# jackBonadies/Guided-Attention

Hardware: AMD Instinct MI355X
Metric: guided images/sec (50-step SD-1.5 512^2) (higher is better)
Workload: dtype f16

## Files before the change

guided-attention_amd/_lib.py:

```python
import ctypes
import os
from pathlib import Path

import torch

_HERE = Path(__file__).resolve().parent
LIB_PATH = Path(os.environ.get("GA_HIP_LIB", _HERE / "libga_hip.so"))

GA_VERSION = 182
GA_F16, GA_BF16, GA_F32 = 0, 1, 2
GA_LINEAR_STREAM = 8
GA_TOK_COOR, GA_TOK_BOX = 0, 1
GA_TERMS = 8
GA_MAX_IMAGES = 64
GA_IMAGE_MAX_TOKENS = 32
DTYPE_CODE = {torch.float16: GA_F16, torch.bfloat16: GA_BF16, torch.float32: GA_F32}


class GaError(RuntimeError):
    pass


class ga_token_t(ctypes.Structure):
    _fields_ = [("token", ctypes.c_int32), ("kind", ctypes.c_int32), ("geom", ctypes.c_double * 4),
                ("weight", ctypes.c_float), ("_pad", ctypes.c_float)]


class ga_loss_params_t(ctypes.Structure):
    _fields_ = [("inside_scale", ctypes.c_float), ("outside_scale", ctypes.c_float), ("center_weight", ctypes.c_float),
                ("sigma", ctypes.c_float), ("shrink", ctypes.c_double), ("ksize", ctypes.c_int32),
                ("smooth", ctypes.c_int32), ("strict", ctypes.c_int32), ("_pad", ctypes.c_int32)]

# ... 56 lines not shown
    "ga_bias_residual_add": [_vp, _vp, _vp, _vp, _i64, _i, _i, _vp],
    "ga_cat_channels": [_vp, _vp, _vp, _i64, _i, _i, _i, _vp],
    "ga_cat_channels_gn_blocks": [_i, _i, _i, _i],
    "ga_linear_gn_blocks": [_i, _i, _i, _i, _i],
    "ga_group_norm_one_launch": [_i, _i, _i, _i],
    "ga_cat_group_norm_fwd": [_vp, _vp, _vp, _vp, _vp, _vp, _vp, _i, _i, _i, _i, _i, _f, _i, _i, _vp],
    "ga_cat_channels_gn": [_vp, _vp, _vp, _vp, _i, _i, _i, _i, _i, _i, _vp],
    "ga_conv3x3_packed_elems": [_i, _i],
    "ga_conv3x3_thin_packed_elems": [_i, _i],
    "ga_conv3x3_thin_supported": [_i, _i, _i, _i],
    "ga_conv3x3_thin_pack": [_vp, _vp, _i, _i, _i64, _i64, _i64, _i64, _i, _i, _vp],
    "ga_conv3x3_thin_in": [_vp, _vp, _vp, _vp, _i, _i, _i, _i, _i, _vp],
    "ga_conv3x3_thin_out": [_vp, _vp, _vp, _vp, _i, _i, _i, _i, _i, _vp],
    "ga_conv3x3_pack_weights": [_vp, _vp, _i, _i, _i64, _i64, _i64, _i64, _i, _i, _vp],
    "ga_conv3x3_plan": [_i, _i, _i, _i, _i, _i, ctypes.POINTER(_i), ctypes.POINTER(_i), ctypes.POINTER(_i),
                        ctypes.POINTER(ctypes.c_longlong)],
    "ga_splitk_workspace_floats": [_i64, _i, _i, _i, _i],
    "ga_conv3x3_nhwc": [_vp, _vp, _vp, _vp, _vp, _vp, _vp, _i, _i, _i, _i, _i, _i, _i, _i, _i, _i, _vp],
    "ga_conv3x3_gn_blocks": [_i, _i, _i, _i, _i, _i],
    "ga_conv3x3_nhwc_gn": [_vp, _vp, _vp, _vp, _vp, _vp, _vp, _i, _i, _i, _i, _i, _i, _i, _i, _i, _vp, _vp, _vp, _i],
    "ga_group_norm_apply": [_vp, _vp, _vp, _vp, _vp, _vp, _vp, _i, _i, _i, _i, _i, _f, _i, _i, _vp],
    "ga_group_norm_two_launch": [_i, _i, _i, _i],
    "ga_conv3x3_up2x_nhwc": [_vp, _vp, _vp, _vp, _vp, _vp, _vp, _i, _i, _i, _i, _i, _i, _i, _i, _i, _vp],
    "ga_gemm_nt": [_vp, _vp, _vp, _vp, _vp, _vp, _vp, _i64, _i, _i, _i, _i, _i, _i, _vp],
    "ga_linear_workspace": [_i64, _i, _i, _i, _i, _i, ctypes.POINTER(ctypes.c_longlong), ctypes.POINTER(_i)],
    "ga_linear_fused": [_vp, _i64, _vp, _vp, _i64, ctypes.POINTER(ga_linear_epilogue_t), _vp, _vp, _i64, _i, _i, _i, _i, _i,
                        _i, _i, _vp],
    "ga_add_layer_norm_fwd": [_vp, _vp, _vp, _vp, _vp, _vp, _vp, _i64, _i, _f, _i, _vp],
    "ga_add_layer_norm_bwd": [_vp, _vp, _vp, _vp, _vp, _vp, _i64, _i, _i, _vp],
}

_lib = None


def load():
    global _lib
    if _lib is None:
        if not LIB_PATH.exists():
            raise GaError(f"{LIB_PATH} not found: build it with `make` (or __graft_entry__.build()); "
                          "the guided-attention path has no CPU fallback")
        lib = ctypes.CDLL(str(LIB_PATH))
        lib.ga_version.argtypes, lib.ga_version.restype = [], ctypes.c_int
        built = lib.ga_version()
        if built != GA_VERSION:
            raise GaError(f"{LIB_PATH} is ABI version {built}, this binding is written for {GA_VERSION}: rebuild with `make`")
        for name, argtypes in PROTOTYPES.items():
# ... 29 lines not shown
```

guided-attention_amd/csrc/conv3x3.hip:

```cpp
#include <cstdlib>

#include "attn_common.h"

using namespace ga;

namespace {

typedef float f32x16 __attribute__((ext_vector_type(16)));
typedef unsigned int u32x4_t __attribute__((ext_vector_type(4)));

#ifndef GA_CONV_PRIO
#define GA_CONV_PRIO 0
#endif
#ifndef GA_CONV_KC
#define GA_CONV_KC 64
#endif
#ifndef GA_CONV_ABL
#define GA_CONV_ABL 0
#endif
constexpr int kKC = GA_CONV_KC;
constexpr int kLD = kKC + 8;
constexpr int kThreads = 256;

template <typename T>
// ... 7 lines not shown
template <>
struct Mma32<bf16_t> {
  __device__ static __forceinline__ f32x16 run(uint4 a, uint4 b, f32x16 c) {
    return __builtin_amdgcn_mfma_f32_32x32x16_bf16(__builtin_bit_cast(bf16x8, a), __builtin_bit_cast(bf16x8, b), c, 0, 0, 0);
  }
};

struct ConvArgs {
  int B, H, W, Cin, Ho, Wo, Cout, stride;
  int M;
  int steps;
  int steps_per;
  int tm, tn;
  int splits;
  int n_fastest;
  int pad;
  int lane_rot;
  unsigned x_bytes, w_bytes;
  int w_tap, w_blk, w_row, w_chunk;
  int pg_nseg, pg_srows;
  int pg_dpr, pg_dpc;
  FastDiv d_tm, d_tn, d_w, d_hw, d_pw, d_segpw, d_segpx, d_wo, d_howo;
  int up;
  float* gn_partials;
  const void* gn_cbias;
  int gn_cg, gn_G, gn_tpi;
};

__device__ __forceinline__ void conv_args_resident(const ConvArgs& a) {
#if defined(__HIP_DEVICE_COMPILE__)
#define GA_TOUCH(x) asm volatile("" ::"s"(x))
  GA_TOUCH(a.B); GA_TOUCH(a.H); GA_TOUCH(a.W); GA_TOUCH(a.Cin); GA_TOUCH(a.Ho); GA_TOUCH(a.Wo); GA_TOUCH(a.Cout); GA_TOUCH(a.stride);
  GA_TOUCH(a.M); GA_TOUCH(a.steps); GA_TOUCH(a.steps_per); GA_TOUCH(a.tm); GA_TOUCH(a.tn); GA_TOUCH(a.splits); GA_TOUCH(a.n_fastest);
  GA_TOUCH(a.pad); GA_TOUCH(a.lane_rot); GA_TOUCH(a.x_bytes); GA_TOUCH(a.w_bytes);
  GA_TOUCH(a.w_tap); GA_TOUCH(a.w_blk); GA_TOUCH(a.w_row); GA_TOUCH(a.w_chunk);
  GA_TOUCH(a.pg_nseg); GA_TOUCH(a.pg_srows); GA_TOUCH(a.pg_dpr); GA_TOUCH(a.pg_dpc);
  GA_TOUCH(a.d_tm.d); GA_TOUCH(a.d_tm.m); GA_TOUCH(a.d_tn.d); GA_TOUCH(a.d_tn.m); GA_TOUCH(a.d_w.d); GA_TOUCH(a.d_w.m);
  GA_TOUCH(a.d_hw.d); GA_TOUCH(a.d_hw.m); GA_TOUCH(a.d_pw.d); GA_TOUCH(a.d_pw.m); GA_TOUCH(a.d_segpw.d); GA_TOUCH(a.d_segpw.m);
  GA_TOUCH(a.d_segpx.d); GA_TOUCH(a.d_segpx.m); GA_TOUCH(a.d_wo.d); GA_TOUCH(a.d_wo.m); GA_TOUCH(a.d_howo.d); GA_TOUCH(a.d_howo.m);
  GA_TOUCH(a.up);
#undef GA_TOUCH
#endif
}

__device__ __forceinline__ unsigned w_row_bytes(const ConvArgs& a, int n, int piece) {
  return (unsigned)(((n >> 6) * a.w_blk + (n & 63) * a.w_row + 8 * piece) * 2);
}
__device__ __forceinline__ unsigned w_step_bytes(const ConvArgs& a, int tap, int chunk) {
  return (unsigned)((tap * a.w_tap + chunk * a.w_chunk) * 2);
}

__device__ __forceinline__ int lane_pixel(int fr, int rot) { return fr < 16 || rot == 0 ? fr : 16 + ((fr - 16 - rot) & 15); }

template <int BM, int BN>
__device__ __forceinline__ void tile_of_workgroup(const ConvArgs& a, int& m0, int& n0, int& split) {
  const int total = a.tm * a.tn * a.splits, q = total >> 3, r = total & 7;
  const int xcd = blockIdx.x & 7, slot = blockIdx.x >> 3;
  const int logical = (xcd < r ? xcd * (q + 1) : r * (q + 1) + (xcd - r) * q) + slot;
  const bool nf = a.n_fastest != 0;
  const FastDiv d1 = nf ? a.d_tn : a.d_tm, d2 = nf ? a.d_tm : a.d_tn;
  const int t1 = nf ? a.tn : a.tm, t2 = nf ? a.tm : a.tn;
  const int rest = fdiv(logical, d1), i1 = logical - rest * t1;
  split = fdiv(rest, d2);
// ... 94 lines not shown
            for (int qd = 0; qd < 4; ++qd)
#pragma unroll
              for (int r = 0; r < 4; ++r)
                acc[j][i][4 * qd + r] += in ? __uint_as_float(v[sb][(j * IM + i) * 4 + qd][r]) : 0.f;
      }
    }
  }
  {
    constexpr int LDC = BN + 8;
    T* Cs = lds;
    float gsum[8] = {0.f, 0.f, 0.f, 0.f, 0.f, 0.f, 0.f, 0.f}, gsq[8] = {0.f, 0.f, 0.f, 0.f, 0.f, 0.f, 0.f, 0.f};
#pragma unroll
    for (int i = 0; i < IM; ++i)
#pragma unroll
      for (int j = 0; j < JN; ++j)
#pragma unroll
        for (int qd = 0; qd < 4; ++qd) {
          typename Traits<T>::frag f;
#pragma unroll
          for (int r = 0; r < 4; ++r) f[r] = Traits<T>::from_f32(acc[j][i][4 * qd + r]);
          store_frag<T>(Cs + (wm * WM + i * 32 + fr) * LDC + wn * WN + j * 32 + 8 * qd + 4 * fh, f);
        }
    __syncthreads();
#pragma unroll
    for (int k = 0; k < NV; ++k) {
      const int r = r0 + k * (kThreads / VPR);
      const int m = m0 + r, n = n0 + cv;
      uint4 val = *reinterpret_cast<const uint4*>(Cs + r * LDC + cv);
      if (bias != nullptr || residual != nullptr) {
        T* e = reinterpret_cast<T*>(&val);
        const T* be = reinterpret_cast<const T*>(&bvec);
        const T* re = reinterpret_cast<const T*>(&rvec[k]);
#pragma unroll
        for (int q = 0; q < 8; ++q)
          e[q] = Traits<T>::from_f32(Traits<T>::to_f32(e[q]) + Traits<T>::to_f32(be[q]) + Traits<T>::to_f32(re[q]));
      }
      if (m < a.M && n < a.Cout) *reinterpret_cast<uint4*>(Y + (size_t)m * a.Cout + n) = val;
      if (gn && m < a.M && n < a.Cout) {
        const T* e = reinterpret_cast<const T*>(&val);
        const T* ge = reinterpret_cast<const T*>(&gvec);
#pragma unroll
        for (int q = 0; q < 8; ++q) {
          const float x = Traits<T>::to_f32(e[q]) + Traits<T>::to_f32(ge[q]);
          gsum[q] += x;
          gsq[q] += x * x;
        }
// ... 61 lines not shown
  __shared__ __attribute__((aligned(16))) T lds[kLds];

  const int tid = threadIdx.x, lane = tid & 63, wave = tid >> 6;
  const int wm = wave >> 1, wn = wave & 1;
  int m0, n0, split;
  conv_args_resident(a);
  tile_of_workgroup<BM, BN>(a, m0, n0, split);
  const int it0 = split * a.steps_per, it1 = min(a.steps, it0 + a.steps_per);
  const int cchunks = a.Cin / kKC;

  constexpr unsigned kOob = 0x80000000u;
  const int srow = tid / QP, sq = tid % QP;
  int a_iy[PA], a_ix[PA];
  int a_off[PA];
#pragma unroll
  for (int p = 0; p < PA; ++p) {
    const int m = m0 + srow + RPP * p;
    const bool ok = m < a.M;
    const int mm = ok ? m : 0;
    const int b = sdiv(mm, a.d_howo), rem = mm - b * (a.Ho * a.Wo);
    const int oy = sdiv(rem, a.d_wo), ox = rem - oy * a.Wo;
    a_iy[p] = ok ? oy * a.stride - a.pad : -4;
    a_ix[p] = ox * a.stride - a.pad;
    a_off[p] = (((b * a.H + a_iy[p]) * a.W + a_ix[p]) * a.Cin + 8 * sq) * (int)sizeof(T);
  }
  unsigned b_off[PB];
#pragma unroll
  for (int p = 0; p < PB; ++p) {
    const int n = n0 + srow + RPP * p;
    b_off[p] = n < a.Cout ? w_row_bytes(a, n, sq) : kOob;
  }
  typedef unsigned int u32x4 __attribute__((ext_vector_type(4)));
  const __amdgpu_buffer_rsrc_t xrsrc = __builtin_amdgcn_make_buffer_rsrc(const_cast<T*>(X), 0, a.x_bytes, 0x00020000);
  const __amdgpu_buffer_rsrc_t wrsrc = __builtin_amdgcn_make_buffer_rsrc(const_cast<T*>(Wp), 0, a.w_bytes, 0x00020000);
  uint4 ra0[PA], rb0[PB], ra1[PA], rb1[PB];
  int ld_it = it0, ld_tap = it0 / cchunks, ld_c = it0 - ld_tap * cchunks;
  int ld_ky = ld_tap / 3, ld_kx = ld_tap - 3 * ld_ky;
  bool in_loop = false;
  auto load_step = [&](uint4 (&ra)[PA], uint4 (&rb)[PB]) {
    if ((GA_CONV_ABL & 1) && in_loop) return;
    const int a_step = ((ld_ky * a.W + ld_kx) * a.Cin + ld_c * kKC) * (int)sizeof(T);
    const unsigned b_step = w_step_bytes(a, ld_tap, ld_c);
#pragma unroll
    for (int p = 0; p < PA; ++p) {
      const bool in = (unsigned)(a_iy[p] + ld_ky) < (unsigned)a.H && (unsigned)(a_ix[p] + ld_kx) < (unsigned)a.W;
      const u32x4 x = __builtin_amdgcn_raw_buffer_load_b128(xrsrc, in ? (unsigned)(a_off[p] + a_step) : kOob, 0, 0);
      ra[p] = uint4{x[0], x[1], x[2], x[3]};
    }
#pragma unroll
    for (int p = 0; p < PB; ++p) {
      const u32x4 x = __builtin_amdgcn_raw_buffer_load_b128(wrsrc, b_off[p] + b_step, 0, 0);
      rb[p] = uint4{x[0], x[1], x[2], x[3]};
    }
    if (ld_it + 1 < it1) {
      ++ld_it;
      if (++ld_c == cchunks) {
        ld_c = 0;
        ++ld_tap;
        if (++ld_kx == 3) {
          ld_kx = 0;
          ++ld_ky;
        }
      }
    }
// ... 130 lines not shown
  if (run) {
    const int in_image = m0 - sdiv(m0, a.d_hw) * hw;
    col0 = in_image - sdiv(in_image, a.d_w) * a.W;
  }
  const int PW = a.W + 2, seg_px = (int)a.d_segpx.d, seg_rows = g.srows + 2, seg_pw = seg_rows * PW;
  const int npatch = g.nseg * seg_pw;

  constexpr unsigned kOob = 0x80000000u;
  const int srow = tid / QP, sq = tid % QP;
  typedef unsigned int u32x4 __attribute__((ext_vector_type(4)));
  const __amdgpu_buffer_rsrc_t xrsrc = __builtin_amdgcn_make_buffer_rsrc(const_cast<T*>(X), 0, a.x_bytes, 0x00020000);
  const __amdgpu_buffer_rsrc_t wrsrc = __builtin_amdgcn_make_buffer_rsrc(const_cast<T*>(Wp), 0, a.w_bytes, 0x00020000);

  unsigned pa_off[kPatchPieces];
#pragma unroll
  for (int p = 0; p < kPatchPieces; ++p) {
    const int q = srow + RPP * p;
    const int seg = sdiv(q, a.d_segpw), rem = q - seg * seg_pw;
    const int pr = sdiv(rem, a.d_pw), pc = rem - pr * PW;
    const int mseg = m0 + seg * seg_px;
    const int b = sdiv(mseg, a.d_hw), y0 = sdiv(mseg - b * hw, a.d_w);
    const int iy = y0 + pr - 1, ix = pc - 1;
    const bool ok = q < npatch && mseg < a.M && (unsigned)iy < (unsigned)a.H && (unsigned)ix < (unsigned)a.W;
    pa_off[p] = ok ? (unsigned)((((b * a.H + iy) * a.W + ix) * a.Cin + 8 * sq) * (int)sizeof(T)) : kOob;
  }
  uint4 rp[kPatchPieces];
  auto load_patch = [&](int chunk) {
    const unsigned step = (unsigned)(chunk * kKC * (int)sizeof(T));
#pragma unroll
    for (int p = 0; p < kPatchPieces; ++p) {
      const u32x4 x = __builtin_amdgcn_raw_buffer_load_b128(xrsrc, pa_off[p] + step, 0, 0);
      rp[p] = uint4{x[0], x[1], x[2], x[3]};
    }
  };
  auto store_patch = [&]() {
#pragma unroll
    for (int p = 0; p < kPatchPieces; ++p)
      *reinterpret_cast<uint4*>(patch + (srow + RPP * p) * kLD + 8 * sq) = rp[p];
  };

  unsigned b_off[PB];
#pragma unroll
  for (int p = 0; p < PB; ++p) {
    const int n = n0 + srow + RPP * p;
    b_off[p] = n < a.Cout ? w_row_bytes(a, n, sq) : kOob;
  }
  constexpr int NS = BN <= 64 ? 9 : 3, PD = BN <= 64 ? 6 : 3;
// ... 186 lines not shown

  PatchGeom g{a.pg_nseg, a.pg_srows};
  const int hw = a.H * a.W;
  const bool run = a.d_segpx.d == (unsigned)BM && BM != g.srows * a.W;
  int col0 = 0;
  if (run) {
    const int in_image = m0 - fdiv(m0, a.d_hw) * hw;
    col0 = in_image - fdiv(in_image, a.d_w) * a.W;
  }
  const int PW = a.W + 2, seg_px = (int)a.d_segpx.d, seg_rows = g.srows + 2, seg_pw = seg_rows * PW;

  constexpr unsigned kOob = 0x80000000u;
  const int srow = tid / QP, sq = tid % QP;
  const __amdgpu_buffer_rsrc_t xrsrc = __builtin_amdgcn_make_buffer_rsrc(const_cast<T*>(X), 0, a.x_bytes, 0x00020000);
  const __amdgpu_buffer_rsrc_t wrsrc = __builtin_amdgcn_make_buffer_rsrc(const_cast<T*>(Wp), 0, a.w_bytes, 0x00020000);
  const unsigned lds0 = (unsigned)(uintptr_t)((__attribute__((address_space(3))) void*)lds);

  unsigned pa_off[kPatchPieces];
  auto patch_offsets = [&]() {
    int seg = fdiv(srow, a.d_segpw);
    const int rem0 = srow - seg * seg_pw;
    int pr = fdiv(rem0, a.d_pw), pc = rem0 - pr * PW;
    const int b0 = fdiv(m0, a.d_hw), y00 = fdiv(m0 - b0 * hw, a.d_w);
    const unsigned row_bytes = (unsigned)(a.Cin * (int)sizeof(T));
    const int SH = a.up ? a.H >> 1 : a.H, SW = a.up ? a.W >> 1 : a.W;
#pragma unroll
    for (int p = 0; p < kPatchPieces; ++p) {
      const int mseg = m0 + seg * seg_px;
      const int b = b0 + seg;
      const int iy = y00 + pr - 1, ix = pc - 1;
      const bool ok = seg < g.nseg && mseg < a.M && (unsigned)iy < (unsigned)a.H && (unsigned)ix < (unsigned)a.W;
      const int sy = a.up ? iy >> 1 : iy, sx = a.up ? ix >> 1 : ix;
      const unsigned pix = __umul24(__umul24((unsigned)b, (unsigned)SH) + (unsigned)sy, (unsigned)SW) + (unsigned)sx;
      pa_off[p] = ok ? __umul24(pix, row_bytes) + (unsigned)(8 * sq * (int)sizeof(T)) : kOob;
      pc += a.pg_dpc;
      pr += a.pg_dpr;
      if (pc >= PW) { pc -= PW; ++pr; }
      if (pr >= seg_rows) { pr -= seg_rows; ++seg; }
      if (pr >= seg_rows) { pr -= seg_rows; ++seg; }
    }
  };
  u32x4_t rp[kPatchPieces];
  auto load_patch = [&](int chunk) {
    const unsigned step = (unsigned)(chunk * kKC * (int)sizeof(T));
#pragma unroll
    for (int p = 0; p < kPatchPieces; ++p) rp[p] = __builtin_amdgcn_raw_buffer_load_b128(xrsrc, pa_off[p] + step, 0, 0);
  };
  const unsigned patch_st = lds0 + (unsigned)((srow * kLD + 8 * sq) * (int)sizeof(T));
  auto store_patch = [&]() {
#pragma unroll
    for (int p = 0; p < kPatchPieces; ++p) conv_lds_write128(patch_st + (unsigned)(RPP * p * kLD * (int)sizeof(T)), rp[p]);
  };

  const int wave_u = __builtin_amdgcn_readfirstlane(wave);
// ... 213 lines not shown
  PatchGeom pg{1, 1};
  const bool geom_ok = a.pad == 1 && a.stride == 1 && (a.W >= 16 || (a.W >= 8 && use_dma() && deep_ring())) && !force_v1();
  const bool patch = geom_ok && patch_geometry(BM, a.H, a.W, pg);
  const bool patch_wide = geom_ok && !patch && (BN <= 64 || BM == 128) && patch_geometry(BM, a.H, a.W, pg, true);
  const bool run_geom = BM % a.W != 0 && BM % (a.H * a.W) != 0;
  const bool dma_wanted = use_dma() && !(run_geom && a.W >= 16);
  bool fast_ok = true;
  {
    const unsigned long long wgs = (unsigned long long)a.tm * a.tn * splits;
    bool map_ok = true;
    a.d_tm = make_fastdiv(a.tm, wgs, map_ok);
    a.d_tn = make_fastdiv(a.tn, wgs, map_ok);
    if (!map_ok) return GA_ERR_SHAPE;
    a.pg_nseg = pg.nseg;
    a.pg_srows = pg.srows;
    const long long seg_px = run_geom ? BM : (long long)pg.srows * a.W, seg_pw = (long long)(pg.srows + 2) * (a.W + 2);
    a.d_w = make_fastdiv(a.W, (unsigned long long)a.H * a.W + seg_px + a.W, fast_ok);
    a.d_hw = make_fastdiv((long long)a.H * a.W, (unsigned long long)a.M + 2ull * BM, fast_ok);
    a.d_pw = make_fastdiv(a.W + 2, (unsigned long long)seg_pw + 512, fast_ok);
    a.d_segpw = make_fastdiv(seg_pw, 1024, fast_ok);
    a.d_segpx = make_fastdiv(seg_px, 2ull * BM, fast_ok);
    a.pg_dpr = 32 / (a.W + 2);
    a.pg_dpc = 32 % (a.W + 2);
    if ((long long)a.B * a.H * a.W >= (1 << 24) || (long long)a.Cin * 2 >= (1 << 24)) fast_ok = false;
    bool tap_ok = true;
    a.d_howo = make_fastdiv((long long)a.Ho * a.Wo, (unsigned long long)a.M + 2ull * BM, tap_ok);
    a.d_wo = make_fastdiv(a.Wo, (unsigned long long)a.Ho * a.Wo, tap_ok);
  }
  const bool dma = dma_wanted && fast_ok;
  if (a.up && !((patch || patch_wide) && dma)) return GA_ERR_SHAPE;
  if (patch_wide) {
    a.steps_per = (a.Cin / kKC + splits - 1) / splits;
    if constexpr (BN <= 64 || BM == 128) {
      if (dma) {
        if (splits == 1)
          hipLaunchKernelGGL((conv3x3_patch_dma_kernel<T, BM, BN, false, true>), grid, dim3(kThreads), 0, s, X, Wp, Y,
                             (float*)nullptr, (unsigned*)nullptr, bias, residual, a);
        else
          hipLaunchKernelGGL((conv3x3_patch_dma_kernel<T, BM, BN, true, true>), grid, dim3(kThreads), 0, s, X, Wp, Y, ws,
                             tickets, bias, residual, a);
      } else if (splits == 1) {
        hipLaunchKernelGGL((conv3x3_patch_kernel<T, BM, BN, false, true>), grid, dim3(kThreads), 0, s, X, Wp, Y,
                           (float*)nullptr, (unsigned*)nullptr, bias, residual, a);
      } else {
        hipLaunchKernelGGL((conv3x3_patch_kernel<T, BM, BN, true, true>), grid, dim3(kThreads), 0, s, X, Wp, Y, ws, tickets,
                           bias, residual, a);
      }
// ... 97 lines not shown
      hipLaunchKernelGGL(conv_pack_kernel<_Float16>, grid, dim3(kThreads), 0, s, (const _Float16*)W, (_Float16*)Wp, Cout, Cin,
                         (long long)stride_o, (long long)stride_i, (long long)stride_y, (long long)stride_x, transpose_flip);
      break;
    case GA_BF16:
      hipLaunchKernelGGL(conv_pack_kernel<bf16_t>, grid, dim3(kThreads), 0, s, (const bf16_t*)W, (bf16_t*)Wp, Cout, Cin,
                         (long long)stride_o, (long long)stride_i, (long long)stride_y, (long long)stride_x, transpose_flip);
      break;
    default:
      return GA_ERR_DTYPE;
  }
  return check_launch();
}

extern "C" int ga_conv3x3_gn_blocks(int H, int W, int Cout, int groups, int bm, int bn) {
  if (H < 1 || W < 1 || groups < 1 || Cout % groups != 0 || (bm != 64 && bm != 128) || (bn != 64 && bn != 128)) return 0;
  const int hw = H * W, cg = Cout / groups;
  if (hw % bm != 0 || cg < 8 || cg > bn || 2 * (hw / bm) > 128) return 0;
  return 2 * (hw / bm);
}

static int conv3x3_nhwc_impl(const void* X, const void* Wp, void* Y, float* workspace, unsigned* tickets, const void* bias,
                             const void* residual, int B, int H, int W, int Cin, int Cout, int stride, int bm, int bn,
                             int splits, int dtype, ga_stream_t stream, float* gn_partials, const void* gn_chan_bias,
                             int gn_groups);

extern "C" int ga_conv3x3_nhwc(const void* X, const void* Wp, void* Y, float* workspace, unsigned* tickets, const void* bias,
                               const void* residual, int B, int H, int W, int Cin, int Cout, int stride, int bm, int bn,
                               int splits, int dtype, ga_stream_t stream) {
  return conv3x3_nhwc_impl(X, Wp, Y, workspace, tickets, bias, residual, B, H, W, Cin, Cout, stride, bm, bn, splits, dtype, stream,
                           nullptr, nullptr, 0);
}

extern "C" int ga_conv3x3_nhwc_gn(const void* X, const void* Wp, void* Y, float* workspace, unsigned* tickets, const void* bias,
                                  const void* residual, int B, int H, int W, int Cin, int Cout, int bm, int bn, int splits,
                                  int dtype, ga_stream_t stream, float* gn_partials, const void* gn_chan_bias, int gn_groups) {
  if (!gn_partials) return GA_ERR_NULL;
  if (ga_conv3x3_gn_blocks(H, W, Cout, gn_groups, bm, bn) == 0) return GA_ERR_UNSUPPORTED;
  if (gn_chan_bias && !al16(gn_chan_bias)) return GA_ERR_ALIGN;
  return conv3x3_nhwc_impl(X, Wp, Y, workspace, tickets, bias, residual, B, H, W, Cin, Cout, 1, bm, bn, splits, dtype, stream,
                           gn_partials, gn_chan_bias, gn_groups);
}

static int conv3x3_nhwc_impl(const void* X, const void* Wp, void* Y, float* workspace, unsigned* tickets, const void* bias,
                             const void* residual, int B, int H, int W, int Cin, int Cout, int stride, int bm, int bn,
                             int splits, int dtype, ga_stream_t stream, float* gn_partials, const void* gn_chan_bias,
                             int gn_groups) {
  if (!X || !Wp || !Y) return GA_ERR_NULL;
  if (B < 1 || H < 1 || W < 1 || Cin < kKC || Cin % kKC != 0 || Cout < 8 || Cout % 8 != 0 || (stride != 1 && stride != 2))
    return GA_ERR_SHAPE;
  if (splits < 1 || splits > 64 || (splits > 1 && (!workspace || !tickets))) return GA_ERR_SHAPE;
  if (!al16(X) || !al16(Wp) || !al16(Y) || (bias && !al16(bias)) || (residual && !al16(residual))) return GA_ERR_ALIGN;
  ConvArgs a;
  a.gn_partials = gn_partials; a.gn_cbias = gn_chan_bias;
  a.gn_G = gn_groups; a.gn_cg = gn_groups ? Cout / gn_groups : 0; a.gn_tpi = gn_groups ? H * W / bm : 0;
  a.B = B; a.H = H; a.W = W; a.Cin = Cin; a.Cout = Cout; a.stride = stride;
  a.Ho = (H - 1) / stride + 1;
  a.Wo = (W - 1) / stride + 1;
  a.M = B * a.Ho * a.Wo;
  a.pad = 1;
  const long long xb = (long long)B * H * W * Cin * 2, wb = ga_conv3x3_packed_elems(Cout, Cin) * 2;
  if (xb >= (1LL << 31) || wb >= (1LL << 31) || (long long)a.M * Cout >= (1LL << 31)) return GA_ERR_SHAPE;
  a.x_bytes = (unsigned)xb;
  a.w_bytes = (unsigned)wb;
  a.w_tap = (int)(wb / 18); a.w_blk = 64 * Cin; a.w_row = 64; a.w_chunk = 64 * kKC;
  a.up = 0;
  hipStream_t s = static_cast<hipStream_t>(stream);
  switch (dtype) {
    case GA_F16: return conv_t<_Float16>(X, Wp, Y, workspace, tickets, bias, residual, a, bm, bn, splits, s);
    case GA_BF16: return conv_t<bf16_t>(X, Wp, Y, workspace, tickets, bias, residual, a, bm, bn, splits, s);
    default: return GA_ERR_DTYPE;
  }
}

extern "C" int ga_conv3x3_up2x_nhwc(const void* X, const void* Wp, void* Y, float* workspace, unsigned* tickets,
                                    const void* bias, const void* residual, int B, int H, int W, int Cin, int Cout, int bm,
                                    int bn, int splits, int dtype, ga_stream_t stream) {
  if (!X || !Wp || !Y) return GA_ERR_NULL;
  if (B < 1 || H < 1 || W < 1 || Cin < kKC || Cin % kKC != 0 || Cout < 8 || Cout % 8 != 0) return GA_ERR_SHAPE;
  if (splits < 1 || splits > 64 || (splits > 1 && (!workspace || !tickets))) return GA_ERR_SHAPE;
  if (!al16(X) || !al16(Wp) || !al16(Y) || (bias && !al16(bias)) || (residual && !al16(residual))) return GA_ERR_ALIGN;
  ConvArgs a;
  a.gn_partials = nullptr; a.gn_cbias = nullptr; a.gn_cg = a.gn_G = a.gn_tpi = 0;
  a.B = B; a.H = 2 * H; a.W = 2 * W; a.Cin = Cin; a.Cout = Cout; a.stride = 1;
  a.Ho = a.H; a.Wo = a.W;
  a.M = B * a.Ho * a.Wo;
  a.pad = 1;
  const long long xb = (long long)B * H * W * Cin * 2, wb = ga_conv3x3_packed_elems(Cout, Cin) * 2;
  if (xb >= (1LL << 31) || wb >= (1LL << 31) || (long long)a.M * Cout >= (1LL << 31)) return GA_ERR_SHAPE;
  a.x_bytes = (unsigned)xb;
  a.w_bytes = (unsigned)wb;
  a.w_tap = (int)(wb / 18); a.w_blk = 64 * Cin; a.w_row = 64; a.w_chunk = 64 * kKC;
  a.up = 1;
  hipStream_t s = static_cast<hipStream_t>(stream);
  switch (dtype) {
    case GA_F16: return conv_t<_Float16>(X, Wp, Y, workspace, tickets, bias, residual, a, bm, bn, splits, s);
    case GA_BF16: return conv_t<bf16_t>(X, Wp, Y, workspace, tickets, bias, residual, a, bm, bn, splits, s);
    default: return GA_ERR_DTYPE;
  }
}

extern "C" int ga_gemm_nt(const void* X, const void* W, void* Y, float* workspace, unsigned* tickets, const void* bias,
                          const void* residual, int64_t M, int K, int N, int bm, int bn, int splits, int dtype,
                          ga_stream_t stream) {
  if (!X || !W || !Y) return GA_ERR_NULL;
  if (M < 1 || K < kKC || K % kKC != 0 || N < 8 || N % 8 != 0) return GA_ERR_SHAPE;
  if (splits < 1 || splits > 64 || (splits > 1 && (!workspace || !tickets))) return GA_ERR_SHAPE;
  if (!al16(X) || !al16(W) || !al16(Y) || (bias && !al16(bias)) || (residual && !al16(residual))) return GA_ERR_ALIGN;
  const long long xb = (long long)M * K * 2, wb = (long long)N * K * 2;
  if (xb >= (1LL << 31) || wb >= (1LL << 31) || (long long)M * N >= (1LL << 31)) return GA_ERR_SHAPE;
  ConvArgs a;
  a.gn_partials = nullptr; a.gn_cbias = nullptr; a.gn_cg = a.gn_G = a.gn_tpi = 0;
  a.B = 1; a.H = (int)M; a.W = 1; a.Cin = K; a.Cout = N; a.stride = 1;
  a.Ho = (int)M; a.Wo = 1; a.M = (int)M;
  a.pad = 0;
  a.x_bytes = (unsigned)xb;
  a.w_bytes = (unsigned)wb;
  a.w_tap = 0; a.w_blk = 64 * K; a.w_row = K; a.w_chunk = kKC;
  a.up = 0;
  hipStream_t s = static_cast<hipStream_t>(stream);
  switch (dtype) {
    case GA_F16: return conv_t<_Float16>(X, W, Y, workspace, tickets, bias, residual, a, bm, bn, splits, s);
    case GA_BF16: return conv_t<bf16_t>(X, W, Y, workspace, tickets, bias, residual, a, bm, bn, splits, s);
    default: return GA_ERR_DTYPE;
  }
}

#if defined(GA_CONV_STAMPS)
extern "C" int ga_conv_set_stamps(void* buffer) {
  unsigned long long* p = static_cast<unsigned long long*>(buffer);
  return hipMemcpyToSymbol(HIP_SYMBOL(g_conv_stamps), &p, sizeof(p)) == hipSuccess ? GA_OK : GA_ERR_LAUNCH;
}
#endif
```

guided-attention_amd/ops.py:

```python
import ctypes
import weakref
from collections import OrderedDict

import torch

from . import _lib
from ._lib import GaError, check, dtype_code, load, require_cuda, stream_ptr


def _ptr(t):
    return ctypes.c_void_p(t.data_ptr()) if t is not None else ctypes.c_void_p(0)


_CENSUS = None


def start_census():
    global _CENSUS
    _CENSUS = {}


def stop_census():
    global _CENSUS
    rec, _CENSUS = _CENSUS, None
# ... 1390 lines not shown
_no_fused_upsample = set()


def conv3x3_up2x_nhwc(x, wp, cout, bias=None, plan=None):
    require_cuda(x, wp, bias)
    x = _nhwc(x)
    B, Cin, H, W = x.shape
    key = (B, H, W, Cin, cout, x.dtype)
    if key in _no_fused_upsample:
        return None
    bm, bn, splits = (plan or conv3x3_plan(B, 2 * H, 2 * W, Cin, cout, 1))[:3]
    y = torch.empty((B, cout, 2 * H, 2 * W), dtype=x.dtype, device=x.device, memory_format=torch.channels_last)
    ws, tickets = splitk_workspace(x.device, B * 4 * H * W, cout, bm, bn, splits)
    rc = load().ga_conv3x3_up2x_nhwc(_ptr(x), _ptr(wp), _ptr(y), _ptr(ws), _ptr(tickets), _ptr(bias), None, B, H, W, Cin,
                                     cout, bm, bn, splits, dtype_code(x), stream_ptr())
    if rc == GA_ERR_SHAPE:
        _no_fused_upsample.add(key)
        return None
    _check_ticketed(rc, "ga_conv3x3_up2x_nhwc", tickets)
    _count(("conv3x3", B, Cin, 4 * H * W, 1, cout, bias is not None, str(x.dtype)))
    return y


class UpsampleConv3x3(torch.autograd.Function):

    @staticmethod
    def forward(ctx, x, weight, bias):
        if ctx.needs_input_grad[1] or (bias is not None and ctx.needs_input_grad[2]):
            raise GaError("convolution weight gradients are not part of the guided-attention path (frozen UNet)")
        y = conv3x3_up2x_nhwc(x, conv3x3_packed_weights(weight, False), weight.shape[0], bias)
        if y is None:
            up = torch.nn.functional.interpolate(x, scale_factor=2.0, mode="nearest")
            y = conv3x3_nhwc(up, conv3x3_packed_weights(weight, False), weight.shape[0], 1, bias)
        ctx.weight, ctx.in_shape = weight, tuple(x.shape)
        return y

    @staticmethod
    def backward(ctx, gy):
        if not ctx.needs_input_grad[0]:
            return None, None, None
        g_up = conv3x3_nhwc(_nhwc(gy), conv3x3_packed_weights(ctx.weight, True), ctx.weight.shape[1], 1)
        B, C, H, W = ctx.in_shape
        gx = torch.ops.aten.upsample_nearest2d_backward(g_up, [2 * H, 2 * W], [B, C, H, W], 2.0, 2.0)
        return gx, None, None


def upsample_conv3x3(x, weight, bias=None):
    return UpsampleConv3x3.apply(x, weight, bias)


class Conv3x3(torch.autograd.Function):

    @staticmethod
    def forward(ctx, x, weight, bias, residual, stride, gn=None):
        if ctx.needs_input_grad[1] or ctx.needs_input_grad[2]:
            raise GaError("convolution weight gradients are not part of the guided-attention path (frozen UNet)")
        wp = conv3x3_packed_weights(weight, False)
        ctx.weight, ctx.stride, ctx.in_shape = weight, stride, tuple(x.shape)
        ctx.has_res = residual is not None
        if gn is None:
            return conv3x3_nhwc(x, wp, weight.shape[0], stride, bias, residual)
        y, made = conv3x3_nhwc(x, wp, weight.shape[0], stride, bias, residual, gn=gn)
        ctx.gn_made = made
        return y

    @staticmethod
    def backward(ctx, gy):
        weight, stride = ctx.weight, ctx.stride
        gx = None
        gy = _nhwc(gy)
        if ctx.needs_input_grad[0]:
            if stride == 1:
                gx = conv3x3_nhwc(gy, conv3x3_packed_weights(weight, True), weight.shape[1], 1)
            else:
                gx = torch.nn.grad.conv2d_input(ctx.in_shape, weight, gy, stride=stride, padding=1)
        return gx, None, None, (gy if ctx.has_res else None), None


def conv3x3(x, weight, bias=None, residual=None, stride=1, gn_for=None):
    if gn_for is None:
        return Conv3x3.apply(x, weight, bias, residual, stride)
    groups, cb = gn_for
    B, _, H, W = x.shape
    cout = weight.shape[0]
    if stride != 1 or not gn_two_launch(H * W, cout, groups, x.dtype):
        return Conv3x3.apply(x, weight, bias, residual, stride)
    box = []
    y = _Conv3x3Gn.apply(x, weight, bias, residual, (groups, cb), box)
    if box and box[0] is not None:
        partials, blocks = box[0]
        y._ga_gn = {"partials": partials, "blocks": blocks, "groups": groups, "chan_bias": cb, "shape": tuple(y.shape),
                    "versions": _gn_versions(y, cb)}
    return y


class _Conv3x3Gn(Conv3x3):

    @staticmethod
# ... 373 lines not shown
```

include/ga_hip.h:

```cpp
#ifndef GA_HIP_H
#define GA_HIP_H

#include <stdint.h>

#ifdef __cplusplus
extern "C" {
#endif

#define GA_VERSION 182

#define GA_MAX_IMAGES 64

typedef void* ga_stream_t;

typedef enum { GA_F16 = 0, GA_BF16 = 1, GA_F32 = 2 } ga_dtype;

typedef enum {
  GA_OK = 0,
  GA_ERR_NULL = -1,
  GA_ERR_SHAPE = -2,
  GA_ERR_DTYPE = -3,
  GA_ERR_ALIGN = -4,
  GA_ERR_LAUNCH = -5,
  GA_ERR_UNSUPPORTED = -6
} ga_status;

int ga_version(void);
const char* ga_strerror(int status);

int ga_attn_capture_fwd(const void* Q, const void* K, const void* V, void* O, void* P,
                        int B, int H, int N, int Kt, int D, float scale, int dtype, ga_stream_t stream);

// ... 134 lines not shown
int ga_cat_group_norm_fwd(const void* a, const void* b, void* cat, const void* gamma, const void* beta, void* y, float* stats,
                          int B, int HW, int C1, int C2, int G, float eps, int act_silu, int dtype, ga_stream_t stream);
int ga_cat_channels_gn_blocks(int HW, int C, int G, int dtype);
int ga_cat_channels_gn(const void* a, const void* b, void* out, float* partials, int B, int HW, int C1, int C2, int G, int dtype,
                       ga_stream_t stream);

long long ga_splitk_workspace_floats(int64_t M, int N, int bm, int bn, int splits);
long long ga_conv3x3_packed_elems(int N, int C);
int ga_conv3x3_pack_weights(const void* W, void* Wp, int Cout, int Cin, int64_t stride_o, int64_t stride_i,
                            int64_t stride_y, int64_t stride_x, int transpose_flip, int dtype, ga_stream_t stream);
int ga_conv3x3_plan(int B, int H, int W, int Cin, int Cout, int stride, int* bm, int* bn, int* splits,
                    long long* workspace_floats);
int ga_conv3x3_nhwc(const void* X, const void* Wp, void* Y, float* workspace, unsigned* tickets, const void* bias,
                    const void* residual, int B, int H, int W, int Cin, int Cout, int stride, int bm, int bn, int splits,
                    int dtype, ga_stream_t stream);
int ga_conv3x3_gn_blocks(int H, int W, int Cout, int groups, int bm, int bn);
int ga_conv3x3_nhwc_gn(const void* X, const void* Wp, void* Y, float* workspace, unsigned* tickets, const void* bias,
                       const void* residual, int B, int H, int W, int Cin, int Cout, int bm, int bn, int splits, int dtype,
                       ga_stream_t stream, float* gn_partials, const void* gn_chan_bias, int gn_groups);

int ga_conv3x3_up2x_nhwc(const void* X, const void* Wp, void* Y, float* workspace, unsigned* tickets, const void* bias,
                         const void* residual, int B, int H, int W, int Cin, int Cout, int bm, int bn, int splits, int dtype,
                         ga_stream_t stream);

long long ga_conv3x3_thin_packed_elems(int Cout, int Cin);
int ga_conv3x3_thin_supported(int H, int W, int Cin, int Cout);
int ga_conv3x3_thin_pack(const void* W, void* Wp, int Cout, int Cin, long long stride_o, long long stride_i, long long stride_y,
                         long long stride_x, int transpose_flip, int dtype, ga_stream_t stream);
int ga_conv3x3_thin_in(const void* X, const void* Wp, const void* bias, void* Y, int B, int H, int W, int Cout, int dtype,
                       ga_stream_t stream);
int ga_conv3x3_thin_out(const void* X, const void* Wp, const void* bias, void* Y, int B, int H, int W, int Cin, int dtype,
                        ga_stream_t stream);

int ga_gemm_nt(const void* X, const void* W, void* Y, float* workspace, unsigned* tickets, const void* bias,
               const void* residual, int64_t M, int K, int N, int bm, int bn, int splits, int dtype, ga_stream_t stream);

#define GA_LINEAR_STREAM 8
typedef struct {
  const void* bias;
  const void* residual;
  int64_t ld_res;
  int geglu;
  void* preact;
  int64_t ld_pre;
  const float* ln_partials;
  int ln_parts;
// ... 26 lines not shown
```

Baseline: 2.011.

## Add fused conv3x3 backward-input kernel with pooled upsample and strided modes

Adds a ga_conv3x3_bwd_input_nhwc entry point that reuses the conv kernel for input gradients. It supports a pixel pitch for strided gradient inputs, zero-insertion for stride-2 backward, and an epilogue that 2x2-sum-pools for the upsample backward. The goal is to avoid separate upsample_nearest2d_backward passes, NHWC copies and the aten conv2d_input fallback. The new modes sit behind Python flags that default to False, so by default only the stride-1 path goes through the new wrapper. That wrapper computes the same thing as before with a little extra host work.

```diff
diff --git a/guided-attention_amd/_lib.py b/guided-attention_amd/_lib.py
--- a/guided-attention_amd/_lib.py
+++ b/guided-attention_amd/_lib.py
@@ -7,7 +7,7 @@
 _HERE = Path(__file__).resolve().parent
 LIB_PATH = Path(os.environ.get("GA_HIP_LIB", _HERE / "libga_hip.so"))
 
-GA_VERSION = 182
+GA_VERSION = 183
 GA_F16, GA_BF16, GA_F32 = 0, 1, 2
 GA_LINEAR_STREAM = 8
 GA_TOK_COOR, GA_TOK_BOX = 0, 1
@@ -110,6 +110,7 @@
     "ga_group_norm_apply": [_vp, _vp, _vp, _vp, _vp, _vp, _vp, _i, _i, _i, _i, _i, _f, _i, _i, _vp],
     "ga_group_norm_two_launch": [_i, _i, _i, _i],
     "ga_conv3x3_up2x_nhwc": [_vp, _vp, _vp, _vp, _vp, _vp, _vp, _i, _i, _i, _i, _i, _i, _i, _i, _i, _vp],
+    "ga_conv3x3_bwd_input_nhwc": [_vp, _i64, _vp, _vp, _vp, _vp, _i, _i, _i, _i, _i, _i, _i, _i, _i, _i, _vp],
     "ga_gemm_nt": [_vp, _vp, _vp, _vp, _vp, _vp, _vp, _i64, _i, _i, _i, _i, _i, _i, _vp],
     "ga_linear_workspace": [_i64, _i, _i, _i, _i, _i, ctypes.POINTER(ctypes.c_longlong), ctypes.POINTER(_i)],
     "ga_linear_fused": [_vp, _i64, _vp, _vp, _i64, ctypes.POINTER(ga_linear_epilogue_t), _vp, _vp, _i64, _i, _i, _i, _i, _i,
diff --git a/guided-attention_amd/csrc/conv3x3.hip b/guided-attention_amd/csrc/conv3x3.hip
--- a/guided-attention_amd/csrc/conv3x3.hip
+++ b/guided-attention_amd/csrc/conv3x3.hip
@@ -53,6 +53,8 @@
   int pg_dpr, pg_dpc;
   FastDiv d_tm, d_tn, d_w, d_hw, d_pw, d_segpw, d_segpx, d_wo, d_howo;
   int up;
+  int x_pitch;
+  int pool;
   float* gn_partials;
   const void* gn_cbias;
   int gn_cg, gn_G, gn_tpi;
@@ -69,7 +71,7 @@
   GA_TOUCH(a.d_tm.d); GA_TOUCH(a.d_tm.m); GA_TOUCH(a.d_tn.d); GA_TOUCH(a.d_tn.m); GA_TOUCH(a.d_w.d); GA_TOUCH(a.d_w.m);
   GA_TOUCH(a.d_hw.d); GA_TOUCH(a.d_hw.m); GA_TOUCH(a.d_pw.d); GA_TOUCH(a.d_pw.m); GA_TOUCH(a.d_segpw.d); GA_TOUCH(a.d_segpw.m);
   GA_TOUCH(a.d_segpx.d); GA_TOUCH(a.d_segpx.m); GA_TOUCH(a.d_wo.d); GA_TOUCH(a.d_wo.m); GA_TOUCH(a.d_howo.d); GA_TOUCH(a.d_howo.m);
-  GA_TOUCH(a.up);
+  GA_TOUCH(a.up); GA_TOUCH(a.x_pitch); GA_TOUCH(a.pool);
 #undef GA_TOUCH
 #endif
 }
@@ -210,6 +212,32 @@
           store_frag<T>(Cs + (wm * WM + i * 32 + fr) * LDC + wn * WN + j * 32 + 8 * qd + 4 * fh, f);
         }
     __syncthreads();
+    if (a.pool) {
+      constexpr int OV = BM / 4 * VPR;
+      const int W2 = a.W >> 1;
+      for (int v = tid; v < OV; v += kThreads) {
+        const int op = v / VPR, c = (v % VPR) * 8;
+        const int orow = sdiv(2 * op, a.d_w), ocol = op - orow * W2;
+        const int r00 = 2 * orow * a.W + 2 * ocol;
+        const uint4 v00 = *reinterpret_cast<const uint4*>(Cs + r00 * LDC + c);
+        const uint4 v01 = *reinterpret_cast<const uint4*>(Cs + (r00 + 1) * LDC + c);
+        const uint4 v10 = *reinterpret_cast<const uint4*>(Cs + (r00 + a.W) * LDC + c);
+        const uint4 v11 = *reinterpret_cast<const uint4*>(Cs + (r00 + a.W + 1) * LDC + c);
+        const T* e00 = reinterpret_cast<const T*>(&v00);
+        const T* e01 = reinterpret_cast<const T*>(&v01);
+        const T* e10 = reinterpret_cast<const T*>(&v10);
+        const T* e11 = reinterpret_cast<const T*>(&v11);
+        uint4 val;
+        T* e = reinterpret_cast<T*>(&val);
+#pragma unroll
+        for (int q = 0; q < 8; ++q)
+          e[q] = Traits<T>::from_f32((Traits<T>::to_f32(e00[q]) + Traits<T>::to_f32(e01[q])) +
+                                     (Traits<T>::to_f32(e10[q]) + Traits<T>::to_f32(e11[q])));
+        const int mo = (m0 >> 2) + op, n = n0 + c;
+        if (mo < (a.M >> 2) && n < a.Cout) *reinterpret_cast<uint4*>(Y + (size_t)mo * a.Cout + n) = val;
+      }
+      return;
+    }
 #pragma unroll
     for (int k = 0; k < NV; ++k) {
       const int r = r0 + k * (kThreads / VPR);
@@ -317,7 +345,7 @@
     const int oy = sdiv(rem, a.d_wo), ox = rem - oy * a.Wo;
     a_iy[p] = ok ? oy * a.stride - a.pad : -4;
     a_ix[p] = ox * a.stride - a.pad;
-    a_off[p] = (((b * a.H + a_iy[p]) * a.W + a_ix[p]) * a.Cin + 8 * sq) * (int)sizeof(T);
+    a_off[p] = (((b * a.H + a_iy[p]) * a.W + a_ix[p]) * a.x_pitch + 8 * sq) * (int)sizeof(T);
   }
   unsigned b_off[PB];
 #pragma unroll
@@ -334,7 +362,7 @@
   bool in_loop = false;
   auto load_step = [&](uint4 (&ra)[PA], uint4 (&rb)[PB]) {
     if ((GA_CONV_ABL & 1) && in_loop) return;
-    const int a_step = ((ld_ky * a.W + ld_kx) * a.Cin + ld_c * kKC) * (int)sizeof(T);
+    const int a_step = ((ld_ky * a.W + ld_kx) * a.x_pitch + ld_c * kKC) * (int)sizeof(T);
     const unsigned b_step = w_step_bytes(a, ld_tap, ld_c);
 #pragma unroll
     for (int p = 0; p < PA; ++p) {
@@ -511,7 +539,7 @@
     const int b = sdiv(mseg, a.d_hw), y0 = sdiv(mseg - b * hw, a.d_w);
     const int iy = y0 + pr - 1, ix = pc - 1;
     const bool ok = q < npatch && mseg < a.M && (unsigned)iy < (unsigned)a.H && (unsigned)ix < (unsigned)a.W;
-    pa_off[p] = ok ? (unsigned)((((b * a.H + iy) * a.W + ix) * a.Cin + 8 * sq) * (int)sizeof(T)) : kOob;
+    pa_off[p] = ok ? (unsigned)((((b * a.H + iy) * a.W + ix) * a.x_pitch + 8 * sq) * (int)sizeof(T)) : kOob;
   }
   uint4 rp[kPatchPieces];
   auto load_patch = [&](int chunk) {
@@ -744,14 +772,15 @@
     const int rem0 = srow - seg * seg_pw;
     int pr = fdiv(rem0, a.d_pw), pc = rem0 - pr * PW;
     const int b0 = fdiv(m0, a.d_hw), y00 = fdiv(m0 - b0 * hw, a.d_w);
-    const unsigned row_bytes = (unsigned)(a.Cin * (int)sizeof(T));
+    const unsigned row_bytes = (unsigned)(a.x_pitch * (int)sizeof(T));
     const int SH = a.up ? a.H >> 1 : a.H, SW = a.up ? a.W >> 1 : a.W;
 #pragma unroll
     for (int p = 0; p < kPatchPieces; ++p) {
       const int mseg = m0 + seg * seg_px;
       const int b = b0 + seg;
       const int iy = y00 + pr - 1, ix = pc - 1;
-      const bool ok = seg < g.nseg && mseg < a.M && (unsigned)iy < (unsigned)a.H && (unsigned)ix < (unsigned)a.W;
+      const bool ok = seg < g.nseg && mseg < a.M && (unsigned)iy < (unsigned)a.H && (unsigned)ix < (unsigned)a.W &&
+                      (a.up != 2 || ((iy | ix) & 1) == 0);
       const int sy = a.up ? iy >> 1 : iy, sx = a.up ? ix >> 1 : ix;
       const unsigned pix = __umul24(__umul24((unsigned)b, (unsigned)SH) + (unsigned)sy, (unsigned)SW) + (unsigned)sx;
       pa_off[p] = ok ? __umul24(pix, row_bytes) + (unsigned)(8 * sq * (int)sizeof(T)) : kOob;
@@ -1011,7 +1040,7 @@
     a.d_segpx = make_fastdiv(seg_px, 2ull * BM, fast_ok);
     a.pg_dpr = 32 / (a.W + 2);
     a.pg_dpc = 32 % (a.W + 2);
-    if ((long long)a.B * a.H * a.W >= (1 << 24) || (long long)a.Cin * 2 >= (1 << 24)) fast_ok = false;
+    if ((long long)a.B * a.H * a.W >= (1 << 24) || (long long)a.x_pitch * 2 >= (1 << 24)) fast_ok = false;
     bool tap_ok = true;
     a.d_howo = make_fastdiv((long long)a.Ho * a.Wo, (unsigned long long)a.M + 2ull * BM, tap_ok);
     a.d_wo = make_fastdiv(a.Wo, (unsigned long long)a.Ho * a.Wo, tap_ok);
@@ -1155,7 +1184,7 @@
 static int conv3x3_nhwc_impl(const void* X, const void* Wp, void* Y, float* workspace, unsigned* tickets, const void* bias,
                              const void* residual, int B, int H, int W, int Cin, int Cout, int stride, int bm, int bn,
                              int splits, int dtype, ga_stream_t stream, float* gn_partials, const void* gn_chan_bias,
-                             int gn_groups);
+                             int gn_groups, long long x_pitch = 0, int up = 0, int pool = 0);
 
 extern "C" int ga_conv3x3_nhwc(const void* X, const void* Wp, void* Y, float* workspace, unsigned* tickets, const void* bias,
                                const void* residual, int B, int H, int W, int Cin, int Cout, int stride, int bm, int bn,
@@ -1177,10 +1206,17 @@
 static int conv3x3_nhwc_impl(const void* X, const void* Wp, void* Y, float* workspace, unsigned* tickets, const void* bias,
                              const void* residual, int B, int H, int W, int Cin, int Cout, int stride, int bm, int bn,
                              int splits, int dtype, ga_stream_t stream, float* gn_partials, const void* gn_chan_bias,
-                             int gn_groups) {
+                             int gn_groups, long long x_pitch, int up, int pool) {
   if (!X || !Wp || !Y) return GA_ERR_NULL;
   if (B < 1 || H < 1 || W < 1 || Cin < kKC || Cin % kKC != 0 || Cout < 8 || Cout % 8 != 0 || (stride != 1 && stride != 2))
     return GA_ERR_SHAPE;
+  if (x_pitch == 0) x_pitch = Cin;
+  if (x_pitch < Cin || x_pitch % 8 != 0 || x_pitch >= (1LL << 30)) return GA_ERR_SHAPE;
+  if ((up || pool) && (stride != 1 || H % 2 != 0 || W % 2 != 0 || bias || residual || gn_partials)) return GA_ERR_SHAPE;
+  if (pool) {
+    const long long hw = (long long)H * W;
+    if (!((bm % (2 * W) == 0 && hw % bm == 0) || bm % hw == 0)) return GA_ERR_SHAPE;
+  }
   if (splits < 1 || splits > 64 || (splits > 1 && (!workspace || !tickets))) return GA_ERR_SHAPE;
   if (!al16(X) || !al16(Wp) || !al16(Y) || (bias && !al16(bias)) || (residual && !al16(residual))) return GA_ERR_ALIGN;
   ConvArgs a;
@@ -1191,12 +1227,13 @@
   a.Wo = (W - 1) / stride + 1;
   a.M = B * a.Ho * a.Wo;
   a.pad = 1;
-  const long long xb = (long long)B * H * W * Cin * 2, wb = ga_conv3x3_packed_elems(Cout, Cin) * 2;
+  const long long x_pixels = up ? (long long)B * (H / 2) * (W / 2) : (long long)B * H * W;
+  const long long xb = ((x_pixels - 1) * x_pitch + Cin) * 2, wb = ga_conv3x3_packed_elems(Cout, Cin) * 2;
   if (xb >= (1LL << 31) || wb >= (1LL << 31) || (long long)a.M * Cout >= (1LL << 31)) return GA_ERR_SHAPE;
   a.x_bytes = (unsigned)xb;
   a.w_bytes = (unsigned)wb;
   a.w_tap = (int)(wb / 18); a.w_blk = 64 * Cin; a.w_row = 64; a.w_chunk = 64 * kKC;
-  a.up = 0;
+  a.up = up; a.x_pitch = (int)x_pitch; a.pool = pool;
   hipStream_t s = static_cast<hipStream_t>(stream);
   switch (dtype) {
     case GA_F16: return conv_t<_Float16>(X, Wp, Y, workspace, tickets, bias, residual, a, bm, bn, splits, s);
@@ -1223,13 +1260,22 @@
   a.x_bytes = (unsigned)xb;
   a.w_bytes = (unsigned)wb;
   a.w_tap = (int)(wb / 18); a.w_blk = 64 * Cin; a.w_row = 64; a.w_chunk = 64 * kKC;
-  a.up = 1;
+  a.up = 1; a.x_pitch = Cin; a.pool = 0;
   hipStream_t s = static_cast<hipStream_t>(stream);
   switch (dtype) {
     case GA_F16: return conv_t<_Float16>(X, Wp, Y, workspace, tickets, bias, residual, a, bm, bn, splits, s);
     case GA_BF16: return conv_t<bf16_t>(X, Wp, Y, workspace, tickets, bias, residual, a, bm, bn, splits, s);
     default: return GA_ERR_DTYPE;
   }
+}
+
+extern "C" int ga_conv3x3_bwd_input_nhwc(const void* GY, int64_t gy_pitch, const void* Wp, void* GX, float* workspace,
+                                         unsigned* tickets, int B, int H, int W, int Cgy, int Cx, int mode, int bm, int bn,
+                                         int splits, int dtype, ga_stream_t stream) {
+  if (mode != GA_CONV_BWD_STRIDE1 && mode != GA_CONV_BWD_STRIDE2 && mode != GA_CONV_BWD_UP2X) return GA_ERR_SHAPE;
+  if (gy_pitch < 1) return GA_ERR_SHAPE;
+  return conv3x3_nhwc_impl(GY, Wp, GX, workspace, tickets, nullptr, nullptr, B, H, W, Cgy, Cx, 1, bm, bn, splits, dtype, stream,
+                           nullptr, nullptr, 0, gy_pitch, mode == GA_CONV_BWD_STRIDE2 ? 2 : 0, mode == GA_CONV_BWD_UP2X ? 1 : 0);
 }
 
 extern "C" int ga_gemm_nt(const void* X, const void* W, void* Y, float* workspace, unsigned* tickets, const void* bias,
@@ -1249,7 +1295,7 @@
   a.x_bytes = (unsigned)xb;
   a.w_bytes = (unsigned)wb;
   a.w_tap = 0; a.w_blk = 64 * K; a.w_row = K; a.w_chunk = kKC;
-  a.up = 0;
+  a.up = 0; a.x_pitch = K; a.pool = 0;
   hipStream_t s = static_cast<hipStream_t>(stream);
   switch (dtype) {
     case GA_F16: return conv_t<_Float16>(X, W, Y, workspace, tickets, bias, residual, a, bm, bn, splits, s);
diff --git a/guided-attention_amd/ops.py b/guided-attention_amd/ops.py
--- a/guided-attention_amd/ops.py
+++ b/guided-attention_amd/ops.py
@@ -1436,6 +1436,50 @@
     return y
 
 
+_OWN_STRIDE2_BWD = False
+_FUSE_UPSAMPLE_BWD = False
+_STRIDED_CONV_GRAD = False
+
+CONV_BWD_STRIDE1, CONV_BWD_STRIDE2, CONV_BWD_UP2X = 0, 1, 2
+_no_own_conv_bwd = set()
+
+
+def _pixel_pitch(g):
+    B, C, H, W = g.shape
+    sb, sc, sh, sw = g.stride()
+    ok = sc == 1 and sw >= C and sw % 8 == 0 and sh == W * sw and (B == 1 or sb == H * W * sw) and g.data_ptr() % 16 == 0
+    return sw if ok else None
+
+
+def conv3x3_bwd_input(gy, weight, mode, plan=None):
+    require_cuda(gy, weight)
+    pitch = _pixel_pitch(gy) if _STRIDED_CONV_GRAD else None
+    if pitch is None:
+        gy = _nhwc(gy)
+        pitch = gy.shape[1]
+    B, Cgy, h, w = gy.shape
+    Cx = weight.shape[1]
+    H, W = (2 * h, 2 * w) if mode == CONV_BWD_STRIDE2 else (h, w)
+    key = (mode, B, H, W, Cgy, Cx, gy.dtype)
+    if key in _no_own_conv_bwd:
+        return None
+    if mode != CONV_BWD_STRIDE1 and (Cgy % CONV_KC != 0 or (mode == CONV_BWD_UP2X and (h % 2 or w % 2))):
+        _no_own_conv_bwd.add(key)
+        return None
+    bm, bn, splits = (plan or conv3x3_plan(B, H, W, Cgy, Cx, 1))[:3]
+    Ho, Wo = (H // 2, W // 2) if mode == CONV_BWD_UP2X else (H, W)
+    gx = torch.empty((B, Cx, Ho, Wo), dtype=gy.dtype, device=gy.device, memory_format=torch.channels_last)
+    ws, tickets = splitk_workspace(gy.device, B * H * W, Cx, bm, bn, splits)
+    rc = load().ga_conv3x3_bwd_input_nhwc(_ptr(gy), pitch, _ptr(conv3x3_packed_weights(weight, True)), _ptr(gx), _ptr(ws),
+                                          _ptr(tickets), B, H, W, Cgy, Cx, mode, bm, bn, splits, dtype_code(gy), stream_ptr())
+    if rc == GA_ERR_SHAPE and mode != CONV_BWD_STRIDE1:
+        _no_own_conv_bwd.add(key)
+        return None
+    _check_ticketed(rc, "ga_conv3x3_bwd_input_nhwc", tickets)
+    _count(("conv3x3", B, Cgy, H * W, 2 if mode == CONV_BWD_STRIDE2 else 1, Cx, False, str(gy.dtype)))
+    return gx
+
+
 class UpsampleConv3x3(torch.autograd.Function):
 
     @staticmethod
@@ -1453,6 +1497,10 @@
     def backward(ctx, gy):
         if not ctx.needs_input_grad[0]:
             return None, None, None
+        if _FUSE_UPSAMPLE_BWD:
+            gx = conv3x3_bwd_input(gy, ctx.weight, CONV_BWD_UP2X)
+            if gx is not None:
+                return gx, None, None
         g_up = conv3x3_nhwc(_nhwc(gy), conv3x3_packed_weights(ctx.weight, True), ctx.weight.shape[1], 1)
         B, C, H, W = ctx.in_shape
         gx = torch.ops.aten.upsample_nearest2d_backward(g_up, [2 * H, 2 * W], [B, C, H, W], 2.0, 2.0)
@@ -1482,12 +1530,17 @@
     def backward(ctx, gy):
         weight, stride = ctx.weight, ctx.stride
         gx = None
-        gy = _nhwc(gy)
+        if not _STRIDED_CONV_GRAD or _pixel_pitch(gy) is None:
+            gy = _nhwc(gy)
         if ctx.needs_input_grad[0]:
             if stride == 1:
-                gx = conv3x3_nhwc(gy, conv3x3_packed_weights(weight, True), weight.shape[1], 1)
+                gx = conv3x3_bwd_input(gy, weight, CONV_BWD_STRIDE1)
             else:
-                gx = torch.nn.grad.conv2d_input(ctx.in_shape, weight, gy, stride=stride, padding=1)
+                H, W = ctx.in_shape[2:]
+                if _OWN_STRIDE2_BWD and H % 2 == 0 and W % 2 == 0:
+                    gx = conv3x3_bwd_input(gy, weight, CONV_BWD_STRIDE2)
+                if gx is None:
+                    gx = torch.nn.grad.conv2d_input(ctx.in_shape, weight, _nhwc(gy), stride=stride, padding=1)
         return gx, None, None, (gy if ctx.has_res else None), None
 
 
diff --git a/include/ga_hip.h b/include/ga_hip.h
--- a/include/ga_hip.h
+++ b/include/ga_hip.h
@@ -7,7 +7,7 @@
 extern "C" {
 #endif
 
-#define GA_VERSION 182
+#define GA_VERSION 183
 
 #define GA_MAX_IMAGES 64
 
@@ -188,6 +188,11 @@
 int ga_conv3x3_up2x_nhwc(const void* X, const void* Wp, void* Y, float* workspace, unsigned* tickets, const void* bias,
                          const void* residual, int B, int H, int W, int Cin, int Cout, int bm, int bn, int splits, int dtype,
                          ga_stream_t stream);
+
+enum { GA_CONV_BWD_STRIDE1 = 0, GA_CONV_BWD_STRIDE2 = 1, GA_CONV_BWD_UP2X = 2 };
+int ga_conv3x3_bwd_input_nhwc(const void* GY, int64_t gy_pitch, const void* Wp, void* GX, float* workspace, unsigned* tickets,
+                              int B, int H, int W, int Cgy, int Cx, int mode, int bm, int bn, int splits, int dtype,
+                              ga_stream_t stream);
 
 long long ga_conv3x3_thin_packed_elems(int Cout, int Cin);
 int ga_conv3x3_thin_supported(int H, int W, int Cin, int Cout);
```

After: 2.000. Within noise of the previous version (-0.5%).
